# Alighieri1231/WaveformInversionUST

Measured on NVIDIA B200. Metric: helmholtz_source_solves_per_sec, higher is better.
Workload: dtype c64

## Files before the change

waveforminversionust_b200/csrc/sweep.cuh:

```cuda
#pragma once
#include "common.cuh"
#include "gemm_simt.cuh"
#include "gemm_tc2.cuh"

namespace ust {

enum SweepMode { SW_ELIM = 0, SW_BACK = 1 };

template <typename R>
struct SweepArgs {
    Geom g;
    int phase, step, nbatch, mode, adjoint, nrhs;
    const cx<R>* planes;
    const cx<R>* T;
    cx<R>* W;
    cx<R>* X;
    size_t x_stride;
    int f0;
    int onehot;
    short first_row[8], last_row[8];
};

template <typename R>
__device__ __forceinline__ bool sweep_tile_is_zero(const SweepArgs<R>& s, int dir, int row, int tn) {
    if (!s.onehot || s.mode != 0  || s.phase != PH_CHAIN || tn >= 8) return false;
    return dir == 0 ? row < s.first_row[tn] : row > s.last_row[tn];
}

struct Coupling { int kind, y, src_row; bool on; };

__device__ __forceinline__ void sweep_couplings(const Geom& g, int mode, int adjoint, int dir, int row, Coupling& lo, Coupling& hi) {
    lo.on = false; hi.on = false;
    lo.src_row = row - 1; hi.src_row = row + 1;
    if (!adjoint) { lo.kind = TRI_L; lo.y = row + 1; hi.kind = TRI_U; hi.y = row + 1; }
    else          { lo.kind = TRI_UC; lo.y = row;    hi.kind = TRI_LC; hi.y = row + 2; }
    const bool has_lo = row > 0, has_hi = row < g.M - 1;
    if (mode == SW_ELIM) {
        if (dir == 0) lo.on = has_lo;
        else if (dir == 1) hi.on = has_hi;
        else { lo.on = has_lo; hi.on = has_hi; }
    } else {
        if (dir == 0) hi.on = has_hi;
        else lo.on = has_lo;
    }
}

template <typename R>
__global__ void __launch_bounds__(256) tri_apply_kernel(SweepArgs<R> s) {
    const int z = blockIdx.z;
    const int row = chain_row(s.g, s.phase, z, s.step);
    if (row < 0) return;
    const int freq = chain_freq(s.phase, z), dir = chain_dir(s.phase, z);
    const int nI = s.g.nI, nrhs = s.nrhs, Nx = s.g.Nx;
    const long long idx = (long long)blockIdx.x * 256 + threadIdx.x;
    if (idx >= (long long)nI * nrhs) return;
    const int a = (int)(idx / nrhs), t = (int)(idx % nrhs);
    const size_t pl = (size_t)s.g.Nx * s.g.Ny;
    const cx<R>* planes_f = s.planes + (size_t)freq * 9 * pl;
    cx<R>* Xf = s.X + (size_t)freq * s.x_stride;
    Coupling lo, hi;
    sweep_couplings(s.g, s.mode, s.adjoint, dir, row, lo, hi);
    cx<R> acc = cxzero<R>();
    Coupling cs[2] = {lo, hi};
#pragma unroll
    for (int c = 0; c < 2; ++c) {
        if (!cs[c].on) continue;
        cx<R> k0, k1, k2;
        tri3<R>(planes_f, s.g, cs[c].kind, s.adjoint != 0, cs[c].y, a, k0, k1, k2);
        const cx<R>* v = Xf + ((size_t)(cs[c].src_row + 1) * Nx + 1) * nrhs;
        if (a > 0) cmac(acc, k0, v[(size_t)(a - 1) * nrhs + t]);
        cmac(acc, k1, v[(size_t)a * nrhs + t]);
        if (a < nI - 1) cmac(acc, k2, v[(size_t)(a + 1) * nrhs + t]);
    }
    cx<R> w;
    if (s.mode == SW_ELIM) {
        cx<R> b = Xf[((size_t)(row + 1) * Nx + 1 + a) * nrhs + t];
        w = b - acc;
    } else {
        w = acc;
    }
    s.W[(size_t)z * s.g.nP * nrhs + (size_t)a * nrhs + t] = w;
}

template <typename R, int BM, int BN, bool TA>
__global__ void __launch_bounds__(256) sweep_gemm_kernel(SweepArgs<R> s) {
    __shared__ GemmSmem<R, BM, BN> sm;
    const int z = blockIdx.z;
    const int row = chain_row(s.g, s.phase, z, s.step);
    if (row < 0) return;
    const int freq = chain_freq(s.phase, z);
    const int nP = s.g.nP, nI = s.g.nI, nrhs = s.nrhs;
    if ((int)blockIdx.y * BM >= nI) return;
    GemmTile<R> t;
    t.A = s.T + ((size_t)freq * s.g.M + row) * (size_t)nP * nP; t.lda = nP;
    t.B = s.W + (size_t)z * nP * nrhs; t.ldb = nrhs;
    cx<R>* out = s.X + (size_t)freq * s.x_stride + ((size_t)(row + 1) * s.g.Nx + 1) * nrhs;
    t.Cin = (s.mode == SW_BACK) ? out : nullptr; t.ldcin = nrhs;
    t.Cout = out; t.ldc = nrhs;
    t.M = nP; t.N = nrhs; t.K = nI; t.Mstore = nI;
    t.m0 = blockIdx.y * BM; t.n0 = blockIdx.x * BN;
    t.mask_lo = 0; t.mask_hi = 0;
    t.sgn = (s.mode == SW_BACK) ? R(-1) : R(1);
    cgemm_tile<R, BM, BN, TA>(t, sm);
}

struct Tc2SweepExtra {
    uint16_t* Wp;
    size_t wp_stride;
    int kpad;
    float bias_fix;
    int drain_every;
    int prefetch_cin;
    int ksplit;
};

__global__ void __launch_bounds__(128) tri_apply2_kernel(SweepArgs<float> s, Tc2SweepExtra x) {
    pdl_trigger();
    pdl_wait();
    typedef float R;
    const int z = blockIdx.z;
    const int row = chain_row(s.g, s.phase, z, s.step);
    if (row < 0) return;
    const int freq = chain_freq(s.phase, z), dir = chain_dir(s.phase, z);
    const int nI = s.g.nI, nrhs = s.nrhs, Nx = s.g.Nx;
    const int kg = blockIdx.x, tn = blockIdx.y, r = threadIdx.x;
    if (sweep_tile_is_zero(s, dir, row, tn)) return;
    const int n = tn * tc2::TN + r;
    const int a0 = kg * 8;
    __shared__ cx<R> coef[2][8][3];
    const size_t pl = (size_t)s.g.Nx * s.g.Ny;
    const cx<R>* planes_f = s.planes + (size_t)freq * 9 * pl;
    Coupling lo, hi;
    sweep_couplings(s.g, s.mode, s.adjoint, dir, row, lo, hi);
    const Coupling cs[2] = {lo, hi};
    const bool active = n < nrhs && a0 < nI;
    const cx<R>* Xf = s.X + (size_t)freq * s.x_stride;
    cx<R> vv[2][10], bb[8];
#pragma unroll
    for (int ci = 0; ci < 2; ++ci) {
        const cx<R>* v = Xf + ((size_t)(cs[ci].src_row + 1) * Nx + 1) * nrhs + n;
#pragma unroll
        for (int c = 0; c < 10; ++c) {
            const int a = a0 - 1 + c;
            vv[ci][c] = (active && cs[ci].on && a >= 0 && a < nI) ? v[(size_t)a * nrhs] : cxzero<R>();
        }
    }
    {
        const cx<R>* b = Xf + ((size_t)(row + 1) * Nx + 1) * nrhs + n;
#pragma unroll
        for (int c = 0; c < 8; ++c) bb[c] = (active && s.mode == SW_ELIM && a0 + c < nI) ? b[(size_t)(a0 + c) * nrhs] : cxzero<R>();
    }
    if (r < 16) {
        const int ci = r >> 3, c = r & 7;
        cx<R> k0 = cxzero<R>(), k1 = cxzero<R>(), k2 = cxzero<R>();
        if (cs[ci].on && a0 + c < nI) tri3<R>(planes_f, s.g, cs[ci].kind, s.adjoint != 0, cs[ci].y, a0 + c, k0, k1, k2);
        coef[ci][c][0] = k0; coef[ci][c][1] = k1; coef[ci][c][2] = k2;
    }
    __syncthreads();
    float re[8], im[8];
#pragma unroll
    for (int c = 0; c < 8; ++c) { re[c] = 0.f; im[c] = 0.f; }
    if (active) {
        cx<R> acc[8];
#pragma unroll
        for (int c = 0; c < 8; ++c) acc[c] = cxzero<R>();
#pragma unroll
        for (int ci = 0; ci < 2; ++ci) {
            if (!cs[ci].on) continue;
#pragma unroll
            for (int c = 0; c < 8; ++c) {
                cmac(acc[c], coef[ci][c][0], vv[ci][c]);
                cmac(acc[c], coef[ci][c][1], vv[ci][c + 1]);
                cmac(acc[c], coef[ci][c][2], vv[ci][c + 2]);
            }
        }
#pragma unroll
        for (int c = 0; c < 8; ++c) {
            const int a = a0 + c;
            if (a >= nI) continue;
            cx<R> w = acc[c];
            if (s.mode == SW_ELIM) w = bb[c] - acc[c];
            re[c] = w.re; im[c] = w.im;
        }
    }
    uint16_t* chunk = x.Wp + (size_t)z * x.wp_stride + ((size_t)tn * (x.kpad / tc2::KC) + (kg >> 1)) * (tc2::B_STAGE / 2);
    tc2::store_b8(chunk, r, kg & 1, re, im);
}

template <bool TA>
__global__ void __launch_bounds__(tc2::NUM_THREADS, 1) tc2_sweep_gemm_kernel(SweepArgs<float> s, Tc2SweepExtra x,
                                                                              const __grid_constant__ CUtensorMap amap) {
    extern __shared__ __align__(1024) unsigned char tc2_smem[];
    pdl_trigger();
    const int z = blockIdx.z;
    const int row = chain_row(s.g, s.phase, z, s.step);
    if (row < 0) { pdl_wait(); return; }
    const int freq = chain_freq(s.phase, z);
    const int nI = s.g.nI, nrhs = s.nrhs;
    const int tn = x.ksplit > 1 ? (int)(blockIdx.x / x.ksplit) : (int)blockIdx.x;
    if (sweep_tile_is_zero(s, chain_dir(s.phase, z), row, tn)) { pdl_wait(); return; }
    tc2::Tc2Tile t;
    tc2::tile_no_emit(t);
    t.bplanes = x.Wp + (size_t)z * x.wp_stride;
    t.amat = (s.f0 + freq) * s.g.M + row;
    cx<float>* out = s.X + (size_t)freq * s.x_stride + ((size_t)(row + 1) * s.g.Nx + 1) * nrhs;
    t.Cin = (s.mode == SW_BACK) ? out : nullptr; t.ldcin = nrhs;
    t.Cout = out; t.ldc = nrhs;
    t.M = nI; t.N = nrhs; t.K = nI; t.Mstore = nI;
    t.m0 = blockIdx.y * tc2::TM; t.n0 = tn * tc2::TN;
    t.mask_lo = 0; t.mask_hi = 0; t.skip_lo = 0; t.skip_hi = 0;
    t.sgn = (s.mode == SW_BACK) ? -1.f : 1.f;
    t.bias_fix = x.bias_fix;
    t.drain_every = x.drain_every;
    t.prefetch_cin = x.prefetch_cin;
    t.ksplit = x.ksplit;
    tc2::cgemm_tile<TA>(t, &amap, tc2_smem);
}

__device__ __forceinline__ int plane_of_offset(int dy, int dx) {
    if (dy == 0) return dx == 0 ? PL_C : (dx < 0 ? PL_L : PL_R);
    if (dy < 0) return dx == 0 ? PL_D : (dx < 0 ? PL_DL : PL_DR);
    return dx == 0 ? PL_U : (dx < 0 ? PL_UL : PL_UR);
}

__device__ __forceinline__ bool ring_node(const Geom& g, int x, int y) { return x == 0 || y == 0 || x == g.Nx - 1 || y == g.Ny - 1; }

__device__ __forceinline__ void inner_ring_node(const Geom& g, int i, int& x, int& y) {
    const int nI = g.nI, M = g.M;
    if (i < nI) { x = 1 + i; y = 1; return; }
    i -= nI;
    if (i < nI) { x = 1 + i; y = M; return; }
    i -= nI;
    if (i < M - 2) { x = 1; y = 2 + i; return; }
    i -= M - 2;
    x = nI; y = 2 + i;
}
__device__ __forceinline__ void outer_ring_node(const Geom& g, int i, int& x, int& y) {
    if (i < g.Nx) { x = i; y = 0; return; }
    i -= g.Nx;
    if (i < g.Nx) { x = i; y = g.Ny - 1; return; }
    i -= g.Nx;
    if (i < g.Ny - 2) { x = 0; y = 1 + i; return; }
    i -= g.Ny - 2;
    x = g.Nx - 1; y = 1 + i;
}

template <typename R>
__global__ void __launch_bounds__(256) ring_pre_kernel(Geom g, const cx<R>* __restrict__ planes_f, cx<R>* __restrict__ X, int nrhs, int count) {
    const long long idx = (long long)blockIdx.x * 256 + threadIdx.x;
    if (idx >= (long long)count * nrhs) return;
    const int i = (int)(idx / nrhs), t = (int)(idx % nrhs);
    int x, y;
    inner_ring_node(g, i, x, y);
    const size_t pl = (size_t)g.Nx * g.Ny;
    cx<R> acc = cxzero<R>();
    for (int dy = -1; dy <= 1; ++dy)
        for (int dx = -1; dx <= 1; ++dx) {
            if (!dx && !dy) continue;
            int xx = x + dx, yy = y + dy;
            if (!ring_node(g, xx, yy)) continue;
            cx<R> c = planes_f[plane_of_offset(dy, dx) * pl + (size_t)y * g.Nx + x];
            cmac(acc, c, X[((size_t)yy * g.Nx + xx) * nrhs + t]);
        }
    size_t o = ((size_t)y * g.Nx + x) * nrhs + t;
    X[o] = X[o] - acc;
}

template <typename R>
__global__ void __launch_bounds__(256) ring_post_adj_kernel(Geom g, const cx<R>* __restrict__ planes_f, cx<R>* __restrict__ X, int nrhs, int count) {
    const long long idx = (long long)blockIdx.x * 256 + threadIdx.x;
    if (idx >= (long long)count * nrhs) return;
    const int i = (int)(idx / nrhs), t = (int)(idx % nrhs);
    int x, y;
    outer_ring_node(g, i, x, y);
    const size_t pl = (size_t)g.Nx * g.Ny;
    cx<R> acc = cxzero<R>();
    for (int dy = -1; dy <= 1; ++dy)
        for (int dx = -1; dx <= 1; ++dx) {
            if (!dx && !dy) continue;
            int xq = x + dx, yq = y + dy;
            if (xq < 1 || yq < 1 || xq > g.Nx - 2 || yq > g.Ny - 2) continue;
            cx<R> c = conj(planes_f[plane_of_offset(-dy, -dx) * pl + (size_t)yq * g.Nx + xq]);
            cmac(acc, c, X[((size_t)yq * g.Nx + xq) * nrhs + t]);
        }
    size_t o = ((size_t)y * g.Nx + x) * nrhs + t;
    X[o] = X[o] - acc;
}

}
```

waveforminversionust_b200/csrc/ustfwi.cu:

```cuda
#include "../../include/ustfwi.h"

#include <math.h>
#include <stdlib.h>
#include <string.h>

#include <algorithm>
#include <map>
#include <mutex>
#include <vector>

#include "assemble.cuh"
#include "common.cuh"
#include "factor.cuh"
#include "fwi.cuh"
#include "sweep.cuh"

namespace ust {
static thread_local std::string g_err;
thread_local long long g_launches = 0;
bool g_use_pdl = true;
thread_local bool g_pdl_batch_ok = true;
void set_error(const std::string& s) { g_err = s; }
}

// ... 304 lines not shown
    if (!p->grid_set) { set_error("ust_factor: ust_plan_set_grid has not been called"); return 1; }
    if (nfreq < 1 || nfreq > p->d.max_freq) { set_error("ust_factor: nfreq out of range"); return 1; }
    UST_CUDA(cudaMemcpyAsync(p->d_freqs, freqs, nfreq * sizeof(double), cudaMemcpyHostToDevice, st));
    if (bde) UST_CUDA(cudaMemcpyAsync(p->d_bde, bde, 3 * nfreq * sizeof(double), cudaMemcpyHostToDevice, st));
    p->freqs_cur.assign(freqs, freqs + nfreq);
    return 0;
}

struct Group { int f0, nf; cudaStream_t st; int idx; };

static std::vector<Group> make_groups(ust_plan* p, int f_begin, int nfreq, cudaStream_t main_st, bool allow_split = true) {
    int G = std::min(std::min(p->ngroups, nfreq / 4), (int)ust_plan::MAX_GROUPS);
    if (p->prof || !allow_split || G < 1) G = 1;
    p->active_groups = G;
    p->eval_nfreq = nfreq;
    std::vector<Group> gs;
    for (int i = 0; i < G; ++i) {
        const int lo = (int)((long long)nfreq * i / G), hi = (int)((long long)nfreq * (i + 1) / G);
        gs.push_back({f_begin + lo, hi - lo, i == 0 ? main_st : p->side[i], i});
    }
    return gs;
}
static int fork_groups(ust_plan* p, const std::vector<Group>& gs) {
    if (gs.size() < 2) return 0;
    UST_CUDA(cudaEventRecord(p->ev_fork, gs[0].st));
    for (size_t i = 1; i < gs.size(); ++i) UST_CUDA(cudaStreamWaitEvent(gs[i].st, p->ev_fork, 0));
    return 0;
}
static int join_groups(ust_plan* p, const std::vector<Group>& gs) {
    for (size_t i = 1; i < gs.size(); ++i) {
        UST_CUDA(cudaEventRecord(p->ev_join[i], gs[i].st));
        UST_CUDA(cudaStreamWaitEvent(gs[0].st, p->ev_join[i], 0));
    }
    return 0;
}

template <typename R>
static int factor_prologue(ust_plan* p, const void* vel_dev, int nfreq, bool has_bde, cudaStream_t st) {
    const Geom& g = p->g;
    if (!has_bde) {
        minmax_kernel<R><<<1, 1024, 0, st>>>((const R*)vel_dev, g.N, p->d_vminmax);
        UST_LAUNCH_CHECK();
        stencil_params_kernel<<<nfreq, 1024, 0, st>>>(p->d_vminmax, p->d_freqs, p->h, p->gr, p->d_bde);
        UST_LAUNCH_CHECK();
    }
    UST_CUDA(cudaMemsetAsync(p->d_status, 0, sizeof(int), st));
    inv_v2_kernel<R><<<(unsigned)((g.N + 255) / 256), 256, 0, st>>>((const R*)vel_dev, p->d_invv2, g.N);
    UST_LAUNCH_CHECK();
    return 0;
}

template <typename R>
static int factor_groups(ust_plan* p, const void* vel_dev, const std::vector<Group>& gs) {
    const Geom& g = p->g;
    AsmArgs aa;
    aa.g = g; aa.h = p->h; aa.gr = p->gr; aa.stencil = p->d.stencil; aa.exp = (p->exp & 8) ? 1 : 0;
    for (const Group& q : gs)
        for (int c0 = 0; c0 < q.nf; c0 += ASM_MAXF) {
            const int f0 = q.f0 + c0;
            aa.nfreq = std::min(q.nf - c0, (int)ASM_MAXF);
            ProfScope ps(p, PC_ASSEMBLE, q.st);
            assemble_kernel<R><<<dim3(cdiv_i(g.Nx, 256), g.Ny), 256, 0, q.st>>>(
                aa, p->d_invv2, (const cx<R>*)p->exn, (const cx<R>*)p->rexh, (const cx<R>*)p->eyn, (const cx<R>*)p->reyh,
                p->d_freqs + f0, p->d_bde + 3 * f0, (cx<R>*)p->planes + (size_t)f0 * 9 * g.N);
            UST_LAUNCH_CHECK();
        }
    const int len = std::max(g.mid, g.M - 1 - g.mid);
    for (int s = 0; s < len; ++s)
        for (const Group& q : gs) UST_TRY(gj_invert_batch<R>(p, PH_CHAIN, s, q.f0, q.nf, q.st, q.idx));
    for (const Group& q : gs) UST_TRY(gj_invert_batch<R>(p, PH_MID, 0, q.f0, q.nf, q.st, q.idx));
    return 0;
}

template <typename R>
static int factor_enqueue(ust_plan* p, const void* vel_dev, int nfreq, bool has_bde, cudaStream_t st) {
    UST_TRY(factor_prologue<R>(p, vel_dev, nfreq, has_bde, st));
    const std::vector<Group> gs = make_groups(p, 0, nfreq, st);
    UST_TRY(fork_groups(p, gs));
    UST_TRY(factor_groups<R>(p, vel_dev, gs));
    UST_TRY(join_groups(p, gs));
    p->nfreq_cur = nfreq;
    p->factored = true;
    return 0;
}

template <typename R>
static int factor_impl(ust_plan* p, const void* vel_dev, int nfreq, const double* freqs, const double* bde, cudaStream_t st) {
    UST_TRY(upload_params(p, nfreq, freqs, bde, st));
    return factor_enqueue<R>(p, vel_dev, nfreq, bde != nullptr, st);
}

template <typename R, int BM, int BN>
static int launch_sweep_gemm(ust_plan* p, const SweepArgs<R>& s, dim3 grid, cudaStream_t st) {
    {
        ProfScope ps(p, PC_SWEEP_GEMM, st);
        if (s.adjoint) sweep_gemm_kernel<R, BM, BN, true><<<grid, 256, 0, st>>>(s);
        else sweep_gemm_kernel<R, BM, BN, false><<<grid, 256, 0, st>>>(s);
    }
    UST_LAUNCH_CHECK();
    return 0;
}

template <typename R>
static int sweep_step(ust_plan* p, SweepArgs<R>& s, cudaStream_t st) {
    const Geom& g = p->g;
    const long long elems = (long long)g.nI * s.nrhs;
    ust::g_pdl_batch_ok = s.nbatch * p->active_groups > p->pdl_min_batch;
    if constexpr (sizeof(R) == 4) {
        if (p->use_tc2) {
            Tc2SweepExtra x;
            x.Wp = p->Wp + (size_t)2 * s.f0 * p->wp_stride;
            x.wp_stride = p->wp_stride; x.kpad = p->kpad; x.bias_fix = p->bias_fix; x.drain_every = p->sweep_drain;
            x.prefetch_cin = p->prefetch_cin; x.ksplit = 1;
            {
                ProfScope ps(p, PC_TRI_APPLY, st);
                UST_CUDA(launch_pdl(tri_apply2_kernel, dim3(p->kpad / 8, cdiv_i(s.nrhs, tc2::TN), s.nbatch), dim3(128), 0, st, s, x));
            }
            UST_LAUNCH_CHECK();
            dim3 grid(cdiv_i(s.nrhs, tc2::TN), cdiv_i(g.nI, tc2::TM), s.nbatch);
            const long long all_tiles = 2LL * p->eval_nfreq * grid.x * grid.y;
            const int nchunks = p->kpad / tc2::KC;
            x.ksplit = 1;
            if (p->ksplit_ok >= 2 && 2 * all_tiles <= p->num_sms && nchunks >= 8) x.ksplit = 2;
            if (p->ksplit_ok >= 4 && 4 * all_tiles <= p->num_sms && nchunks >= 16) x.ksplit = 4;
            {
                ProfScope ps(p, PC_SWEEP_GEMM, st);
                if (x.ksplit > 1) {
                    grid.x *= x.ksplit;
                    if (s.adjoint) UST_CUDA(launch_pdl_cluster(tc2_sweep_gemm_kernel<true>, grid, dim3(tc2::NUM_THREADS), tc2::SMEM_BYTES, st, (unsigned)x.ksplit, s, x, p->amaps[1]));
                    else UST_CUDA(launch_pdl_cluster(tc2_sweep_gemm_kernel<false>, grid, dim3(tc2::NUM_THREADS), tc2::SMEM_BYTES, st, (unsigned)x.ksplit, s, x, p->amaps[0]));
                } else if (s.adjoint) UST_CUDA(launch_pdl(tc2_sweep_gemm_kernel<true>, grid, dim3(tc2::NUM_THREADS), tc2::SMEM_BYTES, st, s, x, p->amaps[1]));
                else UST_CUDA(launch_pdl(tc2_sweep_gemm_kernel<false>, grid, dim3(tc2::NUM_THREADS), tc2::SMEM_BYTES, st, s, x, p->amaps[0]));
            }
            UST_LAUNCH_CHECK();
            return 0;
        }
    }
    {
        ProfScope ps(p, PC_TRI_APPLY, st);
        tri_apply_kernel<R><<<dim3((unsigned)((elems + 255) / 256), 1, s.nbatch), 256, 0, st>>>(s);
    }
    UST_LAUNCH_CHECK();
    const int bn = s.nrhs > 32 ? 64 : 32;
    int bm = 64;
    if ((long long)cdiv_i(g.nI, 64) * cdiv_i(s.nrhs, bn) * s.nbatch < p->num_sms) bm = 32;
    dim3 grid(cdiv_i(s.nrhs, bn), cdiv_i(g.nI, bm), s.nbatch);
    if (bm == 64 && bn == 64) return launch_sweep_gemm<R, 64, 64>(p, s, grid, st);
    if (bm == 32 && bn == 64) return launch_sweep_gemm<R, 32, 64>(p, s, grid, st);
    if (bm == 64 && bn == 32) return launch_sweep_gemm<R, 64, 32>(p, s, grid, st);
    return launch_sweep_gemm<R, 32, 32>(p, s, grid, st);
}

template <typename R>
static int sweeps_groups(ust_plan* p, const std::vector<Group>& gs, cx<R>* X, size_t x_stride, int nrhs, int adjoint, bool onehot = false) {
    const Geom& g = p->g;
    std::vector<SweepArgs<R>> sv(gs.size());
    for (size_t i = 0; i < gs.size(); ++i) {
        SweepArgs<R>& s = sv[i];
        const int f0 = gs[i].f0;
        s.g = g; s.adjoint = adjoint; s.nrhs = nrhs;
        s.onehot = (onehot && p->onehot_ok) ? 1 : 0;
        for (int j = 0; j < 8; ++j) { s.first_row[j] = p->first_row[j]; s.last_row[j] = p->last_row[j]; }
        s.planes = (const cx<R>*)p->planes + (size_t)f0 * 9 * g.N;
        s.T = (const cx<R>*)p->T + (size_t)f0 * g.M * (size_t)g.nP * g.nP;
        s.W = (cx<R>*)p->W + (size_t)2 * f0 * g.nP * p->d.max_nrhs;
        s.X = X + (size_t)f0 * x_stride; s.x_stride = x_stride; s.f0 = f0;
    }
    const int len = std::max(g.mid, g.M - 1 - g.mid);
    for (int step = 0; step < len; ++step)
        for (size_t i = 0; i < gs.size(); ++i) {
            SweepArgs<R>& s = sv[i];
            s.mode = SW_ELIM; s.phase = PH_CHAIN; s.nbatch = 2 * gs[i].nf; s.step = step;
            UST_TRY(sweep_step<R>(p, s, gs[i].st));
        }
    for (size_t i = 0; i < gs.size(); ++i) {
        SweepArgs<R>& s = sv[i];
        s.mode = SW_ELIM; s.phase = PH_MID; s.nbatch = gs[i].nf; s.step = 0;
        UST_TRY(sweep_step<R>(p, s, gs[i].st));
    }
    for (int step = len - 1; step >= 0; --step)
        for (size_t i = 0; i < gs.size(); ++i) {
            SweepArgs<R>& s = sv[i];
            s.mode = SW_BACK; s.phase = PH_CHAIN; s.nbatch = 2 * gs[i].nf; s.step = step;
            UST_TRY(sweep_step<R>(p, s, gs[i].st));
        }
    return 0;
}

template <typename R>
static int ring_fix(ust_plan* p, int ifreq, cx<R>* X, int nrhs, int adjoint, bool before, cudaStream_t st) {
    const Geom& g = p->g;
    const cx<R>* planes_f = (const cx<R>*)p->planes + (size_t)ifreq * 9 * g.N;
    if (!adjoint && before) {
        int count = 2 * g.nI + 2 * std::max(g.M - 2, 0);
        long long th = (long long)count * nrhs;
        ring_pre_kernel<R><<<(unsigned)((th + 255) / 256), 256, 0, st>>>(g, planes_f, X, nrhs, count);
        UST_LAUNCH_CHECK();
    } else if (adjoint && !before) {
        int count = 2 * g.Nx + 2 * (g.Ny - 2);
        long long th = (long long)count * nrhs;
        ring_post_adj_kernel<R><<<(unsigned)((th + 255) / 256), 256, 0, st>>>(g, planes_f, X, nrhs, count);
        UST_LAUNCH_CHECK();
    }
    return 0;
}

template <typename R>
static int solve_impl(ust_plan* p, int ifreq, void* X, int nrhs, int adjoint, cudaStream_t st) {
    if (!p->factored) { set_error("ust_solve: no factorisation (call ust_factor first)"); return 1; }
    if (ifreq < 0 || ifreq >= p->nfreq_cur) { set_error("ust_solve: ifreq out of range"); return 1; }
    if (nrhs < 1 || nrhs > p->d.max_nrhs) { set_error("ust_solve: nrhs exceeds plan max_nrhs"); return 1; }
    UST_TRY(ring_fix<R>(p, ifreq, (cx<R>*)X, nrhs, adjoint, true, st));
    const std::vector<Group> one = {{ifreq, 1, st}};
    UST_TRY(sweeps_groups<R>(p, one, (cx<R>*)X, 0, nrhs, adjoint));
    UST_TRY(ring_fix<R>(p, ifreq, (cx<R>*)X, nrhs, adjoint, false, st));
    return 0;
}

template <bool TA>
__global__ void __launch_bounds__(tc2::NUM_THREADS, 1) tc2_test_gemm_kernel(tc2::Tc2Tile t, const __grid_constant__ CUtensorMap amap) {
    extern __shared__ __align__(1024) unsigned char tc2_smem[];
    t.m0 = blockIdx.y * tc2::TM; t.n0 = blockIdx.x * tc2::TN;
    if (blockIdx.x | blockIdx.y | blockIdx.z) t.trace = nullptr;
    tc2::cgemm_tile<TA>(t, &amap, tc2_smem);
}
__global__ void __launch_bounds__(tc2::NUM_THREADS_H, 2) tc2h_test_gemm_kernel(tc2::Tc2Tile t, const __grid_constant__ CUtensorMap amap) {
    extern __shared__ __align__(1024) unsigned char tc2_smem[];
    t.m0 = blockIdx.y * tc2::TM; t.n0 = blockIdx.x * tc2::TNH;
    if (blockIdx.x | blockIdx.y | blockIdx.z) t.trace = nullptr;
    tc2::cgemm_tile_h(t, &amap, tc2_smem);
}
template <bool TA>
__global__ void __launch_bounds__(256) simt_test_gemm_kernel(GemmTile<float> t) {
    __shared__ GemmSmem<float, 64, 64> sm;
    t.m0 = blockIdx.y * 64; t.n0 = blockIdx.x * 64;
    cgemm_tile<float, 64, 64, TA>(t, sm);
}

__global__ void pack_f32x2_kernel(const double* __restrict__ in, float* __restrict__ out, int n) {
    const int i = blockIdx.x * blockDim.x + threadIdx.x;
    if (i >= n) return;
    const double v = in[i];
    const float hi = (float)v;
    out[2 * i] = hi;
    out[2 * i + 1] = (float)(v - (double)hi);
}

template <typename R>
__global__ void recip_kernel(const R* __restrict__ in, R* __restrict__ out, long long n) {
    long long i = (long long)blockIdx.x * blockDim.x + threadIdx.x;
    if (i < n) out[i] = R(1) / in[i];
}

template <typename R>
static int fwi_enqueue(ust_plan* p, int nfreq, bool has_bde, cudaStream_t st) {
    const Geom& g = p->g;
    const int nt = p->nt;
    const size_t stride = (size_t)g.N * nt;
    const void* slow = p->slow_in;
    double* loss_dev = p->d_scal;
    recip_kernel<R><<<(unsigned)((g.N + 255) / 256), 256, 0, st>>>((const R*)slow, (R*)p->vel, g.N);
    UST_LAUNCH_CHECK();
    UST_TRY(factor_prologue<R>(p, p->vel, nfreq, has_bde, st));
    UST_CUDA(cudaMemsetAsync(loss_dev, 0, sizeof(double), st));
    const std::vector<Group> gs = make_groups(p, 0, nfreq, st);
    UST_TRY(fork_groups(p, gs));
    UST_TRY(factor_groups<R>(p, p->vel, gs));
    for (const Group& q : gs) {
        cx<R>* Uq = (cx<R>*)p->U + (size_t)q.f0 * stride;
        UST_CUDA(cudaMemsetAsync(Uq, 0, stride * q.nf * sizeof(cx<R>), q.st));
        onehot_scatter_kernel<R><<<cdiv_i(nt * q.nf, 256), 256, 0, q.st>>>(Uq, stride, p->src_lin, nt, q.nf);
        UST_LAUNCH_CHECK();
    }
    UST_TRY(sweeps_groups<R>(p, gs, (cx<R>*)p->U, stride, nt, 0, true));
    for (const Group& q : gs) {
        UST_CUDA(cudaMemsetAsync((cx<R>*)p->Lam + (size_t)q.f0 * stride, 0, stride * q.nf * sizeof(cx<R>), q.st));
        RecvArgs<R> ra;
        ra.U = (const cx<R>*)p->U + (size_t)q.f0 * stride; ra.Lam = (cx<R>*)p->Lam + (size_t)q.f0 * stride; ra.stride_f = stride;
        ra.rec = (const cx<R>*)p->rec_in + (size_t)q.f0 * nt * p->nelem;
        ra.rx_lin = p->rx_lin; ra.mask = p->mask; ra.src_est = (cx<R>*)p->src_est + (size_t)q.f0 * nt; ra.loss = loss_dev;
        ra.nt = nt; ra.nm = p->nm; ra.nelem = p->nelem;
        ProfScope ps(p, PC_RECEIVER, q.st);
        receiver_kernel<R><<<dim3(nt, q.nf), 256, 0, q.st>>>(ra);
        UST_LAUNCH_CHECK();
    }
    UST_TRY(sweeps_groups<R>(p, gs, (cx<R>*)p->Lam, stride, nt, 1));
    for (const Group& q : gs)
        for (int f = q.f0; f < q.f0 + q.nf; ++f) UST_TRY(ring_fix<R>(p, f, (cx<R>*)p->Lam + (size_t)f * stride, nt, 1, false, q.st));
    UST_TRY(join_groups(p, gs));
    GradArgs<R> ga;
    ga.U = (const cx<R>*)p->U; ga.Lam = (const cx<R>*)p->Lam; ga.stride_f = stride; ga.src_est = (const cx<R>*)p->src_est;
    ga.freqs = p->d_freqs; ga.slow = (const R*)slow; ga.grad = (R*)p->grad_out; ga.N = g.N; ga.nt = nt; ga.nfreq = nfreq;
    const int blocks = (int)std::min<long long>((g.N + 7) / 8, (long long)p->num_sms * 8);
    {
        ProfScope ps(p, PC_GRADIENT, st);
        gradient_kernel<R><<<blocks, 256, 0, st>>>(ga);
    }
    UST_LAUNCH_CHECK();
    return 0;
}

template <typename R>
static int linesearch_enqueue(ust_plan* p, cudaStream_t st) {
    const Geom& g = p->g;
    const int nt = p->nt, nfreq = p->nfreq_cur;
    const size_t stride = (size_t)g.N * nt;
    double* out2 = p->d_scal + 2;
    UST_CUDA(cudaMemsetAsync(out2, 0, 2 * sizeof(double), st));
    const std::vector<Group> gs = make_groups(p, 0, nfreq, st);
    UST_TRY(fork_groups(p, gs));
    for (const Group& q : gs) {
        PertArgs<R> pa;
        pa.U = (const cx<R>*)p->U + (size_t)q.f0 * stride; pa.Out = (cx<R>*)p->Lam + (size_t)q.f0 * stride; pa.stride_f = stride;
        pa.src_est = (const cx<R>*)p->src_est + (size_t)q.f0 * nt;
        pa.freqs = p->d_freqs + q.f0; pa.slow = (const R*)p->slow_in; pa.sd = (const R*)p->sd_in; pa.N = g.N; pa.nt = nt; pa.nfreq = q.nf;
        pert_rhs_kernel<R><<<dim3(p->num_sms * 4, q.nf), 256, 0, q.st>>>(pa);
        UST_LAUNCH_CHECK();
    }
    UST_TRY(sweeps_groups<R>(p, gs, (cx<R>*)p->Lam, stride, nt, 0));
    for (const Group& q : gs) {
        LineArgs<R> la;
        la.U = (const cx<R>*)p->U + (size_t)q.f0 * stride; la.Pert = (const cx<R>*)p->Lam + (size_t)q.f0 * stride; la.stride_f = stride;
        la.rec = (const cx<R>*)p->rec_in + (size_t)q.f0 * nt * p->nelem;
        la.rx_lin = p->rx_lin; la.mask = p->mask; la.src_est = (const cx<R>*)p->src_est + (size_t)q.f0 * nt; la.out2 = out2;
        la.nt = nt; la.nm = p->nm; la.nelem = p->nelem;
        linesearch_kernel<R><<<dim3(nt, q.nf), 256, 0, q.st>>>(la);
        UST_LAUNCH_CHECK();
    }
    UST_TRY(join_groups(p, gs));
    return 0;
}

template <typename F>
static int run_graphed(ust_plan* p, long long key, cudaStream_t user, F enqueue) {
    if (!p->use_graphs || p->prof) return enqueue(user);
    cudaStream_t gs = p->own_stream;
    auto it = p->graphs.find(key);
    if (it == p->graphs.end()) {
        const long long before = ust::g_launches;
        UST_CUDA(cudaStreamBeginCapture(gs, cudaStreamCaptureModeThreadLocal));
        int rc = enqueue(gs);
        cudaGraph_t graph = nullptr;
        cudaError_t e = cudaStreamEndCapture(gs, &graph);
        if (rc || e != cudaSuccess || !graph) {
            if (graph) cudaGraphDestroy(graph);
            if (!rc) set_error(std::string("CUDA graph capture failed: ") + cudaGetErrorString(e));
            cudaGetLastError();
            return 1;
        }
        ust_plan::GraphEntry ge;
        ge.launches = ust::g_launches - before;
        ust::g_launches = before;
        e = cudaGraphInstantiate(&ge.exec, graph, 0);
        cudaGraphDestroy(graph);
        if (e != cudaSuccess) { set_error(std::string("cudaGraphInstantiate failed: ") + cudaGetErrorString(e)); return 1; }
        it = p->graphs.emplace(key, ge).first;
    }
    UST_CUDA(cudaEventRecord(p->ev_in, user));
    UST_CUDA(cudaStreamWaitEvent(gs, p->ev_in, 0));
    UST_CUDA(cudaGraphLaunch(it->second.exec, gs));
    UST_CUDA(cudaEventRecord(p->ev_out, gs));
    UST_CUDA(cudaStreamWaitEvent(user, p->ev_out, 0));
    ust::g_launches += it->second.launches;
    return 0;
}

template <typename R>
static int fwi_impl(ust_plan* p, const void* slow, const void* rec, int nfreq, const double* freqs, const double* bde,
                    double* loss_dev, void* grad_dev, cudaStream_t st) {
    const Geom& g = p->g;
    if (!p->acq_set) { set_error("ust_fwi_loss_grad: ust_plan_set_acquisition has not been called"); return 1; }
    if (!p->U) { set_error("ust_fwi_loss_grad: plan was created with fwi_buffers=0"); return 1; }
    if (p->nt > p->d.max_nrhs) { set_error("ust_fwi_loss_grad: nt exceeds plan max_nrhs"); return 1; }
    UST_TRY(upload_params(p, nfreq, freqs, bde, st));
    if (slow != p->slow_in) UST_CUDA(cudaMemcpyAsync(p->slow_in, slow, g.N * sizeof(R), cudaMemcpyDeviceToDevice, st));
    if (rec != p->rec_in) UST_CUDA(cudaMemcpyAsync(p->rec_in, rec, (size_t)nfreq * p->nt * p->nelem * sizeof(cx<R>), cudaMemcpyDeviceToDevice, st));
    const bool has_bde = bde != nullptr;
    const long long key = 1000LL * nfreq + (has_bde ? 1 : 0);
    UST_TRY(run_graphed(p, key, st, [&](cudaStream_t s_) { return fwi_enqueue<R>(p, nfreq, has_bde, s_); }));
    p->nfreq_cur = nfreq;
    p->factored = true;
    UST_CUDA(cudaMemcpyAsync(loss_dev, p->d_scal, sizeof(double), cudaMemcpyDeviceToDevice, st));
    UST_CUDA(cudaMemcpyAsync(grad_dev, p->grad_out, g.N * sizeof(R), cudaMemcpyDeviceToDevice, st));
    p->fwi_done = true;
    if (p->trace) return dump_update_trace(p, st);
    return 0;
}

template <typename R>
static int linesearch_impl(ust_plan* p, const void* sd, double* out2, cudaStream_t st) {
    const Geom& g = p->g;
    if (!p->factored || !p->fwi_done) { set_error("ust_ncg_linesearch: call ust_fwi_loss_grad first"); return 1; }
    UST_CUDA(cudaMemcpyAsync(p->sd_in, sd, g.N * sizeof(R), cudaMemcpyDeviceToDevice, st));
    const long long key = 1000LL * p->nfreq_cur + 500;
    UST_TRY(run_graphed(p, key, st, [&](cudaStream_t s_) { return linesearch_enqueue<R>(p, s_); }));
    UST_CUDA(cudaMemcpyAsync(out2, p->d_scal + 2, 2 * sizeof(double), cudaMemcpyDeviceToDevice, st));
    return 0;
}

template <typename R>
static int set_kernel_attrs() {
    UST_CUDA(cudaFuncSetAttribute(gj_pivot_kernel<R>, cudaFuncAttributeMaxDynamicSharedMemorySize,
                                  (int)std::max(gj_pivot_smem<R>(), sizeof(R) == 4 ? gj_pivot2_smem_bytes : gj_pivot_f64_smem_bytes)));
    if (sizeof(R) == 4) UST_CUDA(cudaFuncSetAttribute(gj_k0_kernel, cudaFuncAttributeMaxDynamicSharedMemorySize, (int)gj_pivot2_smem_bytes));
    if (sizeof(R) == 4) UST_CUDA(cudaFuncSetAttribute(schur_kernel<float>, cudaFuncAttributeMaxDynamicSharedMemorySize, (int)gj_pivot2_scratch_bytes));

    UST_CUDA(cudaFuncSetAttribute(gj_rowpanel_kernel<R>, cudaFuncAttributeMaxDynamicSharedMemorySize, (int)gj_rowpanel_smem<R>()));
    if (sizeof(R) == 4) {
        UST_CUDA(cudaFuncSetAttribute(tc2_sweep_gemm_kernel<true>, cudaFuncAttributeMaxDynamicSharedMemorySize, tc2::SMEM_BYTES));
        UST_CUDA(cudaFuncSetAttribute(tc2_sweep_gemm_kernel<false>, cudaFuncAttributeMaxDynamicSharedMemorySize, tc2::SMEM_BYTES));
        UST_CUDA(cudaFuncSetAttribute(tc2_gj_update_kernel, cudaFuncAttributeMaxDynamicSharedMemorySize, tc2::SMEM_BYTES_H));
        UST_CUDA(cudaFuncSetAttribute(tc2_gj_rowpanel_kernel, cudaFuncAttributeMaxDynamicSharedMemorySize, tc2::SMEM_BYTES_H));
        UST_CUDA(cudaFuncSetAttribute(tc2_gj_pivot_deep_kernel, cudaFuncAttributeMaxDynamicSharedMemorySize, tc2::SMEM_BYTES_H));
        UST_CUDA(cudaFuncSetAttribute(tc2_gj2_rowpanel_kernel, cudaFuncAttributeMaxDynamicSharedMemorySize, tc2::SMEM_BYTES_H));
        UST_CUDA(cudaFuncSetAttribute(tc2_gj2_update_kernel, cudaFuncAttributeMaxDynamicSharedMemorySize, tc2::SMEM_BYTES_H));
        UST_CUDA(cudaFuncSetAttribute(gj2_k0_kernel, cudaFuncAttributeMaxDynamicSharedMemorySize, (int)gj_pivot2_smem_bytes));
        UST_CUDA(cudaFuncSetAttribute(tc2h_test_gemm_kernel, cudaFuncAttributeMaxDynamicSharedMemorySize, tc2::SMEM_BYTES_H));
        UST_CUDA(cudaFuncSetAttribute(tc2_test_gemm_kernel<true>, cudaFuncAttributeMaxDynamicSharedMemorySize, tc2::SMEM_BYTES));
        UST_CUDA(cudaFuncSetAttribute(tc2_test_gemm_kernel<false>, cudaFuncAttributeMaxDynamicSharedMemorySize, tc2::SMEM_BYTES));
    }
    return 0;
}

#define DISPATCH(p, fn, ...) ((p)->d.dtype == UST_C64 ? fn<float>(__VA_ARGS__) : fn<double>(__VA_ARGS__))

struct IdtftCache { void* buf = nullptr; size_t cap = 0; cudaEvent_t ev = nullptr; bool used = false; };

template <typename R>
static int idtft_impl(const void* U, int nf, long long npix, const double* freqs, const double* resp, double df, const double* time, int nt,
                      void* out, cudaStream_t st) {
    const double PI = 3.14159265358979323846;
    std::vector<cx<R>> w((size_t)nt * nf);
    for (int t = 0; t < nt; ++t)
        for (int k = 0; k < nf; ++k) {
            const double ph = 2.0 * PI * freqs[k] * time[t], a = df * (resp ? resp[k] : 1.0);
            w[(size_t)t * nf + k] = cx<R>((R)(a * cos(ph)), (R)(a * sin(ph)));
        }
    int dev = 0;
    UST_CUDA(cudaGetDevice(&dev));
    static std::mutex mu;
    static std::map<int, IdtftCache> caches;
    std::lock_guard<std::mutex> lock(mu);
    IdtftCache& c = caches[dev];
    const size_t need = w.size() * sizeof(cx<R>);
    if (!c.ev) UST_CUDA(cudaEventCreateWithFlags(&c.ev, cudaEventDisableTiming));
    if (need > c.cap) {
        if (c.buf) { UST_CUDA(cudaEventSynchronize(c.ev)); cudaFree(c.buf); c.buf = nullptr; c.cap = 0; }
        UST_CUDA(cudaMalloc(&c.buf, need));
        c.cap = need;
    } else if (c.used) {
        UST_CUDA(cudaStreamWaitEvent(st, c.ev, 0));
    }
    cx<R>* wd = (cx<R>*)c.buf;
    UST_CUDA(cudaMemcpyAsync(wd, w.data(), need, cudaMemcpyHostToDevice, st));
    const size_t smem = (size_t)IDTFT_TT * nf * sizeof(cx<R>);
    if (smem > 48 * 1024) UST_CUDA(cudaFuncSetAttribute(idtft_kernel<R>, cudaFuncAttributeMaxDynamicSharedMemorySize, (int)smem));
    idtft_kernel<R><<<dim3((unsigned)((npix + 255) / 256), (unsigned)cdiv_i(nt, IDTFT_TT)), 256, smem, st>>>((const cx<R>*)U, wd, (cx<R>*)out, npix, nf, nt);
    UST_LAUNCH_CHECK();
    UST_CUDA(cudaEventRecord(c.ev, st));
    c.used = true;
    return 0;
}

extern "C" {

const char* ust_last_error(void) { return g_err.c_str(); }
const char* ust_version(void) { return "ustfwi 0.1 (sm_100a)"; }
int ust_idtft(int dtype, const void* U_dev, int nf, long long npix, const double* freqs, const double* resp, double df,
              const double* time, int nt, void* out_dev, void* stream) {
    if (!U_dev || !out_dev || !freqs || !time) { set_error("ust_idtft: null argument"); return 1; }
    if (nf < 1 || nt < 1 || npix < 1) { set_error("ust_idtft: empty problem"); return 1; }
    if ((size_t)IDTFT_TT * nf * (dtype == UST_C64 ? 8 : 16) > 200 * 1024) { set_error("ust_idtft: too many frequencies for one pass (split the stack)"); return 1; }
// ... 506 lines not shown
```

Baseline: 28770.

## Overlap tri-apply RHS and coefficient loads with PDL wait, specialize on couplings

Result: no change. 29040 (median of 6 runs) (+0.9%).

```diff
diff --git a/waveforminversionust_b200/csrc/sweep.cuh b/waveforminversionust_b200/csrc/sweep.cuh
--- a/waveforminversionust_b200/csrc/sweep.cuh
+++ b/waveforminversionust_b200/csrc/sweep.cuh
@@ -19,6 +19,7 @@
     int f0;
     int onehot;
     short first_row[8], last_row[8];
+    int rhs_early;
 };
 
 template <typename R>
@@ -114,49 +115,38 @@
     int ksplit;
 };
 
-__global__ void __launch_bounds__(128) tri_apply2_kernel(SweepArgs<float> s, Tc2SweepExtra x) {
-    pdl_trigger();
+template <int NC, bool GUARD>
+__device__ __forceinline__ void tri_apply2_rows(const SweepArgs<float>& s, const Coupling (&cs)[2], const cx<float>* planes_f,
+                                                const cx<float>* Xf, int row, int n, int a0, uint16_t* chunk, int kh) {
+    typedef float R;
+    const int nI = s.g.nI, nrhs = s.nrhs, Nx = s.g.Nx, r = threadIdx.x;
+    const bool elim = s.mode == SW_ELIM;
+    const bool active = !GUARD || (n < nrhs && a0 < nI);
+    __shared__ __align__(16) cx<R> coef[NC > 0 ? NC : 1][8][3];
+    cx<R> vv[NC > 0 ? NC : 1][10], bb[8];
+    if (elim) {
+        const cx<R>* b = Xf + ((size_t)(row + 1) * Nx + 1 + a0) * nrhs + n;
+#pragma unroll
+        for (int c = 0; c < 8; ++c, b += nrhs) bb[c] = (!GUARD || (active && a0 + c < nI)) ? *b : cxzero<R>();
+    }
+    if (r < 8 * NC) {
+        const int ci = r >> 3, c = r & 7;
+        const Coupling& cc = ci ? cs[NC - 1] : cs[0];
+        cx<R> k0 = cxzero<R>(), k1 = cxzero<R>(), k2 = cxzero<R>();
+        if (!GUARD || a0 + c < nI) tri3<R>(planes_f, s.g, cc.kind, s.adjoint != 0, cc.y, a0 + c, k0, k1, k2);
+        coef[ci][c][0] = k0; coef[ci][c][1] = k1; coef[ci][c][2] = k2;
+    }
     pdl_wait();
-    typedef float R;
-    const int z = blockIdx.z;
-    const int row = chain_row(s.g, s.phase, z, s.step);
-    if (row < 0) return;
-    const int freq = chain_freq(s.phase, z), dir = chain_dir(s.phase, z);
-    const int nI = s.g.nI, nrhs = s.nrhs, Nx = s.g.Nx;
-    const int kg = blockIdx.x, tn = blockIdx.y, r = threadIdx.x;
-    if (sweep_tile_is_zero(s, dir, row, tn)) return;
-    const int n = tn * tc2::TN + r;
-    const int a0 = kg * 8;
-    __shared__ cx<R> coef[2][8][3];
-    const size_t pl = (size_t)s.g.Nx * s.g.Ny;
-    const cx<R>* planes_f = s.planes + (size_t)freq * 9 * pl;
-    Coupling lo, hi;
-    sweep_couplings(s.g, s.mode, s.adjoint, dir, row, lo, hi);
-    const Coupling cs[2] = {lo, hi};
-    const bool active = n < nrhs && a0 < nI;
-    const cx<R>* Xf = s.X + (size_t)freq * s.x_stride;
-    cx<R> vv[2][10], bb[8];
-#pragma unroll
-    for (int ci = 0; ci < 2; ++ci) {
-        const cx<R>* v = Xf + ((size_t)(cs[ci].src_row + 1) * Nx + 1) * nrhs + n;
-#pragma unroll
-        for (int c = 0; c < 10; ++c) {
+#pragma unroll
+    for (int ci = 0; ci < NC; ++ci) {
+        const cx<R>* v = Xf + ((size_t)(cs[ci].src_row + 1) * Nx + a0) * nrhs + n;
+#pragma unroll
+        for (int c = 0; c < 10; ++c, v += nrhs) {
             const int a = a0 - 1 + c;
-            vv[ci][c] = (active && cs[ci].on && a >= 0 && a < nI) ? v[(size_t)a * nrhs] : cxzero<R>();
-        }
-    }
-    {
-        const cx<R>* b = Xf + ((size_t)(row + 1) * Nx + 1) * nrhs + n;
-#pragma unroll
-        for (int c = 0; c < 8; ++c) bb[c] = (active && s.mode == SW_ELIM && a0 + c < nI) ? b[(size_t)(a0 + c) * nrhs] : cxzero<R>();
-    }
-    if (r < 16) {
-        const int ci = r >> 3, c = r & 7;
-        cx<R> k0 = cxzero<R>(), k1 = cxzero<R>(), k2 = cxzero<R>();
-        if (cs[ci].on && a0 + c < nI) tri3<R>(planes_f, s.g, cs[ci].kind, s.adjoint != 0, cs[ci].y, a0 + c, k0, k1, k2);
-        coef[ci][c][0] = k0; coef[ci][c][1] = k1; coef[ci][c][2] = k2;
-    }
-    __syncthreads();
+            vv[ci][c] = (!GUARD || (active && a >= 0 && a < nI)) ? *v : cxzero<R>();
+        }
+    }
+    if (NC > 0) __syncthreads();
     float re[8], im[8];
 #pragma unroll
     for (int c = 0; c < 8; ++c) { re[c] = 0.f; im[c] = 0.f; }
@@ -165,8 +155,7 @@
 #pragma unroll
         for (int c = 0; c < 8; ++c) acc[c] = cxzero<R>();
 #pragma unroll
-        for (int ci = 0; ci < 2; ++ci) {
-            if (!cs[ci].on) continue;
+        for (int ci = 0; ci < NC; ++ci) {
 #pragma unroll
             for (int c = 0; c < 8; ++c) {
                 cmac(acc[c], coef[ci][c][0], vv[ci][c]);
@@ -176,15 +165,42 @@
         }
 #pragma unroll
         for (int c = 0; c < 8; ++c) {
-            const int a = a0 + c;
-            if (a >= nI) continue;
+            if (GUARD && a0 + c >= nI) continue;
             cx<R> w = acc[c];
-            if (s.mode == SW_ELIM) w = bb[c] - acc[c];
+            if (elim) w = bb[c] - acc[c];
             re[c] = w.re; im[c] = w.im;
         }
     }
+    tc2::store_b8(chunk, r, kh, re, im);
+}
+
+__global__ void __launch_bounds__(128, 6) tri_apply2_kernel(SweepArgs<float> s, Tc2SweepExtra x) {
+    pdl_trigger();
+    if (!s.rhs_early || s.mode != SW_ELIM) pdl_wait();
+    const int z = blockIdx.z;
+    const int row = chain_row(s.g, s.phase, z, s.step);
+    if (row < 0) { pdl_wait(); return; }
+    const int freq = chain_freq(s.phase, z), dir = chain_dir(s.phase, z);
+    const int nI = s.g.nI;
+    const int kg = blockIdx.x, tn = blockIdx.y;
+    if (sweep_tile_is_zero(s, dir, row, tn)) { pdl_wait(); return; }
+    const int n = tn * tc2::TN + threadIdx.x;
+    const int a0 = kg * 8;
+    const size_t pl = (size_t)s.g.Nx * s.g.Ny;
+    const cx<float>* planes_f = s.planes + (size_t)freq * 9 * pl;
+    const cx<float>* Xf = s.X + (size_t)freq * s.x_stride;
     uint16_t* chunk = x.Wp + (size_t)z * x.wp_stride + ((size_t)tn * (x.kpad / tc2::KC) + (kg >> 1)) * (tc2::B_STAGE / 2);
-    tc2::store_b8(chunk, r, kg & 1, re, im);
+    Coupling lo, hi;
+    sweep_couplings(s.g, s.mode, s.adjoint, dir, row, lo, hi);
+    Coupling cs[2] = {lo, hi};
+    if (!lo.on) cs[0] = hi;
+    const int nc = (int)lo.on + (int)hi.on;
+    const bool interior = a0 >= 1 && a0 + 8 < nI && (tn + 1) * tc2::TN <= s.nrhs;
+    if (interior && nc == 1) tri_apply2_rows<1, false>(s, cs, planes_f, Xf, row, n, a0, chunk, kg & 1);
+    else if (interior && nc == 2) tri_apply2_rows<2, false>(s, cs, planes_f, Xf, row, n, a0, chunk, kg & 1);
+    else if (nc == 1) tri_apply2_rows<1, true>(s, cs, planes_f, Xf, row, n, a0, chunk, kg & 1);
+    else if (nc == 2) tri_apply2_rows<2, true>(s, cs, planes_f, Xf, row, n, a0, chunk, kg & 1);
+    else tri_apply2_rows<0, true>(s, cs, planes_f, Xf, row, n, a0, chunk, kg & 1);
 }
 
 template <bool TA>
diff --git a/waveforminversionust_b200/csrc/ustfwi.cu b/waveforminversionust_b200/csrc/ustfwi.cu
--- a/waveforminversionust_b200/csrc/ustfwi.cu
+++ b/waveforminversionust_b200/csrc/ustfwi.cu
@@ -480,7 +480,8 @@
 }
 
 template <typename R>
-static int sweeps_groups(ust_plan* p, const std::vector<Group>& gs, cx<R>* X, size_t x_stride, int nrhs, int adjoint, bool onehot = false) {
+static int sweeps_groups(ust_plan* p, const std::vector<Group>& gs, cx<R>* X, size_t x_stride, int nrhs, int adjoint, bool onehot = false,
+                         bool rhs_early = false) {
     const Geom& g = p->g;
     std::vector<SweepArgs<R>> sv(gs.size());
     for (size_t i = 0; i < gs.size(); ++i) {
@@ -488,6 +489,7 @@
         const int f0 = gs[i].f0;
         s.g = g; s.adjoint = adjoint; s.nrhs = nrhs;
         s.onehot = (onehot && p->onehot_ok) ? 1 : 0;
+        s.rhs_early = rhs_early ? 1 : 0;
         for (int j = 0; j < 8; ++j) { s.first_row[j] = p->first_row[j]; s.last_row[j] = p->last_row[j]; }
         s.planes = (const cx<R>*)p->planes + (size_t)f0 * 9 * g.N;
         s.T = (const cx<R>*)p->T + (size_t)f0 * g.M * (size_t)g.nP * g.nP;
@@ -600,7 +602,7 @@
         onehot_scatter_kernel<R><<<cdiv_i(nt * q.nf, 256), 256, 0, q.st>>>(Uq, stride, p->src_lin, nt, q.nf);
         UST_LAUNCH_CHECK();
     }
-    UST_TRY(sweeps_groups<R>(p, gs, (cx<R>*)p->U, stride, nt, 0, true));
+    UST_TRY(sweeps_groups<R>(p, gs, (cx<R>*)p->U, stride, nt, 0, true, true));
     for (const Group& q : gs) {
         UST_CUDA(cudaMemsetAsync((cx<R>*)p->Lam + (size_t)q.f0 * stride, 0, stride * q.nf * sizeof(cx<R>), q.st));
         RecvArgs<R> ra;
@@ -612,7 +614,7 @@
         receiver_kernel<R><<<dim3(nt, q.nf), 256, 0, q.st>>>(ra);
         UST_LAUNCH_CHECK();
     }
-    UST_TRY(sweeps_groups<R>(p, gs, (cx<R>*)p->Lam, stride, nt, 1));
+    UST_TRY(sweeps_groups<R>(p, gs, (cx<R>*)p->Lam, stride, nt, 1, false, true));
     for (const Group& q : gs)
         for (int f = q.f0; f < q.f0 + q.nf; ++f) UST_TRY(ring_fix<R>(p, f, (cx<R>*)p->Lam + (size_t)f * stride, nt, 1, false, q.st));
     UST_TRY(join_groups(p, gs));
@@ -645,7 +647,7 @@
         pert_rhs_kernel<R><<<dim3(p->num_sms * 4, q.nf), 256, 0, q.st>>>(pa);
         UST_LAUNCH_CHECK();
     }
-    UST_TRY(sweeps_groups<R>(p, gs, (cx<R>*)p->Lam, stride, nt, 0));
+    UST_TRY(sweeps_groups<R>(p, gs, (cx<R>*)p->Lam, stride, nt, 0, false, true));
     for (const Group& q : gs) {
         LineArgs<R> la;
         la.U = (const cx<R>*)p->U + (size_t)q.f0 * stride; la.Pert = (const cx<R>*)p->Lam + (size_t)q.f0 * stride; la.stride_f = stride;
```
